# KumarRobotics/top_down_renderer

Measured on AMD Instinct MI355X. Metric: particle-updates/sec (render+score+resample), higher is better.
Workload: dtype f32

## Files before the change

### include/tdr.h

```cpp
#ifndef TDR_H_
#define TDR_H_

#include <stddef.h>
#include <stdint.h>

#ifdef __cplusplus
extern "C" {
#endif

#define TDR_OK 0
#define TDR_ERR_ARG (-1)
#define TDR_ERR_HIP (-2)
#define TDR_ERR_NOMEM (-3)

#define TDR_MAX_CLASSES 15
#define TDR_ST_FIELDS 7
enum { TDR_ST_INIT_X = 0, TDR_ST_INIT_Y = 1, TDR_ST_DX = 2, TDR_ST_DY = 3, TDR_ST_THETA = 4, TDR_ST_SCALE = 5,
       TDR_ST_HAVE_INIT = 6 };

typedef struct tdr_state {
  float init_x_px, init_y_px, dx_m, dy_m, theta, scale;
  uint8_t have_init;
  uint8_t pad_[3];
} tdr_state;
// ... 152 lines not shown

#define TDR_UW_INFO_FLOATS 65536
int tdr_k_update_weights(const float* raw_w, const float* last_dist, int64_t n, float* w_out, float* info_out,
                         void* stream);

int tdr_config_prefix_small(int on);
int64_t tdr_prefix_workspace_bytes(int64_t n);
int tdr_k_prefix(const float* w, int64_t n, float* runmax_out, void* workspace, void* stream);
int tdr_k_prefix_mode(const float* w, int64_t n, int mode, float* runmax_out, float* prefix_out, void* workspace,
                      void* stream);
int tdr_k_resample(const float* runmax, int64_t n, int64_t n_new, float shift, int64_t i_begin, int64_t i_end,
                   int32_t* idx_out, void* stream);
int tdr_k_resample_dev(const float* runmax, int64_t n, int64_t n_new, const float* shift_dev, int64_t i_begin, int64_t i_end,
                       int32_t* idx_out, void* stream);
int tdr_k_gather_states(const float* src, int64_t src_cap, int64_t src_shard, const int32_t* idx, int64_t n_new,
                        float* dst, int64_t dst_cap, void* stream);

int tdr_k_shard_pack2(const float* a, const float* b, int64_t nl, float* out, void* stream);
int tdr_k_shard_unpack2(const float* in, int world, int64_t nl, float* a_glob, float* b_glob, void* stream);
int tdr_k_unshard_states(const float* in, int world, int64_t nl, float* st, int64_t cap, void* stream);

int tdr_k_local_map_polar(const tdr_map_desc* map, const float* tab, int nb, int nr, float cx, float cy, float scale,
                          float res, float* dists_out, uint8_t* mask_out, void* stream);
int tdr_k_local_map_cart(const tdr_map_desc* map, int rows, int cols, float cx, float cy, float rot, float res,
                         float* dists_out, uint8_t* mask_out, void* stream);

int tdr_k_active_diffs(const tdr_map_desc* map, const float* tab, int nb, int nr, float res, const float* centres,
                       const int32_t* shifts, int K, int ncand, double* sums_out, void* stream);
int tdr_active_candidates_host(const float* preds, int K, int nb, float* centres, float* dists, float* thetas,
                               int32_t* shifts, int* ntheta_out, int* ndist_out);

#define TDR_MEAN_COV_FLOATS 4800
int tdr_k_mean_cov(const float* st, int64_t cap, int64_t n, const float* about, float* out, void* stream);
int tdr_k_set_scale(float* st, int64_t cap, int64_t n, const float* scale_dev, void* stream);
int tdr_k_save_ml_state(const float* info, const float* st, int64_t cap, int64_t src_shard, int64_t n, float* out12,
                        void* stream);
int tdr_k_shift_init(float* st, int64_t cap, int64_t n, float dx, float dy, void* stream);
int tdr_k_resample_gather(const float* runmax, int64_t n, int64_t n_new, const float* shift_dev, float shift,
                          int64_t i_begin, int64_t i_end, int32_t* idx_out, const float* src, int64_t src_cap,
                          int64_t src_shard, float* dst, int64_t dst_cap, const float* info, float* out12, void* stream);

int tdr_config_compact(int on);
int tdr_config_shift_uniform(int mode);
float tdr_config_shift_uniform_span(float cells);
int tdr_config_ray_split(int k);
int tdr_config_cart_skip(int on);
int tdr_config_init_mfma(int on);
int tdr_config_uw_waves(int on);
int64_t tdr_shift_uniform_launches(void);

int tdr_profile_enable(int on);
int tdr_profile_score_ms(double* total_ms, int64_t* launches);
int tdr_profile_shares(double* dense_ms, double* scattered_ms, int64_t* scattered_particles);
int tdr_profile_variants(int64_t out[16]);
int tdr_profile_ray_gate(int64_t out[4]);
int tdr_profile_su_list(int64_t out[2]);

int64_t tdr_config_tuning(const char* name, int64_t value);
int tdr_su_tail_plan(int nchunks, int k, int q, int row, int* group, int* s0, int* s1);
size_t tdr_k_su_order_workspace_ints(int64_t n, int nb);
int64_t tdr_k_su_order_slots(int64_t n, int nb);
int tdr_k_su_order(const float* st, int64_t cap, int64_t n, const int32_t* perm, int nb, float span, int32_t* workspace,
                   int32_t* slots_out, int32_t* keys_out, int32_t* counts_out, int* bucket_out, void* stream);
int tdr_k_score_prep(const tdr_map_desc* map, const float* tab, const float* scan_pk, int nb, int nr, float res,
                     const float* st, int64_t cap, int64_t n, int64_t n_total, const int32_t* perm, float uniform_scale,
                     float span, float* workspace, tdr_score_ctx* ctx, int64_t* layout, void* const* out, void* stream);
int tdr_k_score_prep_full_mask(const tdr_map_desc* map, int nb, int nr, int64_t n, int64_t n_total, const float* workspace,
                               uint32_t* out, int64_t* words, void* stream);
int tdr_selftest_score(void);
int tdr_k_selftest_round(const float* x, int64_t n, float limit, int32_t* out, void* stream);
int tdr_libm_variant(void);
int tdr_libm_force_variant(int variant);
int tdr_sincosf_host(const float* x, int64_t n, int variant, float* sin_out, float* cos_out);
int tdr_k_selftest_sincos(const float* x, int64_t n, float* sin_out, float* cos_out, void* stream);
int tdr_logf_host(const float* x, int64_t n, float* out);
int tdr_k_selftest_logf(const float* x, int64_t n, float* out, void* stream);
int tdr_k_selftest_atan2(const float* y, const float* x, int64_t n, float* out, void* stream);

int tdr_k_states_aos_to_soa(const tdr_state* aos, int64_t n, float* st, int64_t cap, void* stream);
int tdr_k_states_soa_to_aos(const float* st, int64_t cap, int64_t n, tdr_state* aos, void* stream);
size_t tdr_locality_tmp_ints(int64_t n, int map_rows, int map_cols);
int tdr_k_locality_order(const float* st, int64_t cap, int64_t n, int map_rows, int map_cols, int32_t* perm_out,
                         int32_t* keys_tmp, void* stream);
size_t tdr_locality_pose_tmp_ints(int64_t n);
int tdr_k_locality_order_pose(const float* st, int64_t cap, int64_t n, int map_rows, int map_cols, float theta_radius,
                              int32_t* perm_out, int32_t* keys_tmp, void* stream);

typedef struct tdr_map tdr_map;
typedef struct tdr_renderer tdr_renderer;
typedef struct tdr_filter tdr_filter;

int tdr_map_create(tdr_map** out);
void tdr_map_destroy(tdr_map* m);
int tdr_map_set(tdr_map* m, const float* class_maps, const uint8_t* class_mask, int ncls, int rows, int cols,
                float resolution, int center_x, int center_y);
int tdr_map_set_labels(tdr_map* m, const uint8_t* label_img, int img_h, int img_w, const int32_t* flatten_lut,
                       int lut_size, int ncls, float resolution, int center_x, int center_y);
int tdr_map_update_labels_incremental(tdr_map* m, const uint8_t* label_img, int img_h, int img_w,
                                      const int32_t* flatten_lut, int lut_size, int ncls, float resolution, int center_x,
                                      int center_y, int64_t* changed_cells);
int tdr_map_patch_labels(tdr_map* m, const uint8_t* patch, int y0, int x0, int h, int w, int center_x, int center_y,
                         int64_t* changed_cells);
int tdr_map_get_desc(const tdr_map* m, tdr_map_desc* out);
int tdr_map_sample_pts_polar(tdr_map* m, int nb, int nr, float ang_res);
int tdr_map_polar_shape(const tdr_map* m, int* nb, int* nr);
int tdr_map_set_window(tdr_map* m, int rows, int cols);
int tdr_map_window_shape(const tdr_map* m, int* rows, int* cols);
int tdr_map_info(const tdr_map* m, int* ncls, int* rows, int* cols, float* resolution, int* have_map);
int tdr_map_center(const tdr_map* m, int* center_x, int* center_y);
int tdr_map_local_map(tdr_map* m, int polar, float cx, float cy, float scale_or_rot, float res, int rows, int cols,
                      float* dists_out, uint8_t* mask_out);
int tdr_map_classes_at_point(const tdr_map* m, int px, int py, uint32_t* class_bits);
int tdr_map_best_rel_pos(tdr_map* m, const float* preds, int K, float best_rel_pos[2], float* best_diff);
int tdr_map_local_geo_map(tdr_map* m, int polar, float cx, float cy, float scale_or_rot, float res, int rows, int cols,
                          float* dists_out);
int tdr_map_load_cache(tdr_map* m, const char* cache_dir, const char* map_path, int num_classes, float resolution,
                       int center_x, int center_y, int* loaded);
int tdr_map_save_cache(tdr_map* m, const char* cache_dir, const char* map_path);
int tdr_map_save_rasters(tdr_map* m, const char* dir);
int tdr_png_read_gray8_host(const char* path, uint8_t* px_out, int64_t capacity, int* w, int* h);
int tdr_png_write_gray8_host(const char* path, const uint8_t* px, int w, int h);
int tdr_map_load_rasters(tdr_map* m, const char* dir, int num_classes, float resolution, int center_x, int center_y);
#define TDR_SVG_NO_KEY 0xFFFFFFFFu
int tdr_svg_parse_host(const char* path, float size_out[2], int64_t* n_poly, int64_t* n_vert, uint32_t* keys_out,
                       int64_t* offsets_out, float* verts_out);
int tdr_map_load_polygons(tdr_map* m, const float* verts, const int64_t* poly_offsets, const int32_t* poly_class,
                          int64_t n_poly, int width, int height, int num_classes, const int32_t* exclusive, int n_excl,
                          float resolution, int center_x, int center_y, uint8_t* planes_out);
int tdr_polygon_planes(const float* verts, const int64_t* poly_offsets, const int32_t* poly_class, int64_t n_poly,
                       int width, int height, int num_classes, const int32_t* exclusive, int n_excl, float resolution,
                       uint8_t* planes_out);
int tdr_map_load_svg(tdr_map* m, const char* path, const uint32_t* fill_keys, const int32_t* flatten_lut, int lut_size,
                     int num_classes, const int32_t* exclusive, int n_excl, float resolution, int center_x, int center_y);
int tdr_png_read_color_host(const char* path, uint8_t* bgr_out, int64_t capacity, int* w, int* h);
int tdr_map_load_color_image(tdr_map* m, const uint8_t* bgr, int img_h, int img_w, const uint32_t* fill_keys,
                             const int32_t* flatten_lut, int lut_size, int num_classes, float resolution, int center_x,
                             int center_y);
int tdr_map_load_color_png(tdr_map* m, const char* path, const uint32_t* fill_keys, const int32_t* flatten_lut,
                           int lut_size, int num_classes, float resolution, int center_x, int center_y);

int tdr_renderer_create(const int32_t* flatten_lut256, tdr_renderer** out);
void tdr_renderer_destroy(tdr_renderer* r);
int tdr_renderer_render(tdr_renderer* r, int polar, const float* pts, int stride, int ioff, int64_t n, float res,
                        float ang_res, int ncls, int rows, int cols, float* imgs_out);

int tdr_renderer_render_geo(tdr_renderer* r, int polar, const float* pts, int stride, int64_t width, int64_t height,
                            float res, float ang_res, int rows, int cols, float* imgs_out);

#define TDR_COMM_ID_BYTES 128
typedef struct tdr_comm tdr_comm;
typedef struct tdr_comm_ops {
  void* ctx;
  int (*all_gather)(void* ctx, const void* send_dev, void* recv_dev, size_t bytes_per_rank, void* stream);
  int (*broadcast)(void* ctx, void* buf_dev, size_t bytes, int root, void* stream);
} tdr_comm_ops;
int tdr_comm_rccl_unique_id(void* id_out128);
int tdr_comm_create_rccl(int world_size, int rank, const void* unique_id128, tdr_comm** out);
int tdr_comm_create(int world_size, int rank, const tdr_comm_ops* ops, tdr_comm** out);
void tdr_comm_destroy(tdr_comm* c);
int tdr_comm_world(const tdr_comm* c);
int tdr_comm_rank(const tdr_comm* c);
int tdr_comm_all_gather(tdr_comm* c, const void* send_dev, void* recv_dev, size_t bytes_per_rank, void* stream);
int tdr_comm_broadcast(tdr_comm* c, void* buf_dev, size_t bytes, int root, void* stream);
int tdr_filter_create_sharded(tdr_map* map, int n_max, const tdr_filter_params* fp, uint32_t seed, tdr_comm* comm,
                              tdr_filter** out);
int64_t tdr_filter_num_local(const tdr_filter* f);
// ... 280 lines not shown
```

### top_down_renderer_amd/_lib.py

```python
import ctypes as C
import os

_PKG = os.path.dirname(os.path.abspath(__file__))
SO_PATH = os.environ.get("TDR_LIB_PATH") or os.path.join(_PKG, "libtdr_hip.so")

TDR_ST_FIELDS = 7
TDR_MAX_CLASSES = 15
TDR_SVG_NO_KEY = 0xFFFFFFFF


class FilterParamsC(C.Structure):
    _fields_ = [
        ("pos_cov", C.c_float), ("theta_cov", C.c_float), ("regularization", C.c_float),
        ("init_pos_px_x", C.c_float), ("init_pos_px_y", C.c_float), ("init_pos_px_cov", C.c_float),
        ("init_pos_m_x", C.c_float), ("init_pos_m_y", C.c_float),
        ("init_pos_deg_theta", C.c_float), ("init_pos_deg_cov", C.c_float),
        ("force_on_map", C.c_int32),
        ("fixed_scale", C.c_float), ("scale_log_min", C.c_float), ("scale_log_max", C.c_float),
        ("num_classes", C.c_int32),
        ("class_weights", C.c_float * 16),
    ]


class MapDescC(C.Structure):
# ... 308 lines not shown
    "tdr_filter_get_resample_indices": (_i, [_vp, _vp, _i64]),
    "tdr_filter_mean_cov": (_i, [_vp, _i, _vp, _vp]),
    "tdr_filter_freeze_scale": (_i, [_vp]),
    "tdr_filter_is_scale_frozen": (_i, [_vp]),
    "tdr_filter_scale": (_f, [_vp]),
    "tdr_filter_num_particles": (_i64, [_vp]),
    "tdr_filter_update_map": (_i, [_vp, _vp, _vp, _i, _i, _i, _f, _i, _i]),
    "tdr_batch_step": (_i, [_vp, _i, _vp, _vp]),
    "tdr_batch_last_stats": (_i, [_vp, _vp]),
    "tdr_batch_render_polar": (_i, [_vp, _i, _vp, _f, _i, _i, _i, _vp]),
    "tdr_renderer_get_render": (_i, [_vp, _vp, _vp]),
    "tdr_batch_pose": (_i, [_vp, _i, _vp, _vp]),
    "tdr_viz_plane_words": (C.c_size_t, [_i, _i]),
    "tdr_viz_arrow_host": (_i, [_i, _i, _vp]),
    "tdr_viz_overlay_host": (_i, [_vp, _vp, _i, _vp, _vp, _i, _i, _vp, _i, C.POINTER(_i)]),
    "tdr_k_viz_particles": (_i, [_vp, _i64, _i64, _i, _i, _vp, _vp]),
    "tdr_k_viz_segments": (_i, [_vp, _i, _i, _i, _vp, _vp]),
    "tdr_k_viz_compose": (_i, [_vp, _i, _i, _vp, _i, _i, _vp, _vp]),
    "tdr_filter_set_viz_background": (_i, [_vp, _vp, _i, _i]),
    "tdr_filter_visualize": (_i, [_vp, _f, _vp, _i, _vp, _i64, C.POINTER(_i), C.POINTER(_i)]),
    "tdr_k_viz_particles_jobs": (_i, [_vp, _i, _i64, _vp]),
    "tdr_k_viz_segments_jobs": (_i, [_vp, _i, _i, _vp]),
    "tdr_k_viz_compose_jobs": (_i, [_vp, _i, _i64, _vp]),
    "tdr_batch_visualize": (_i, [_vp, _i, _f, _vp, _vp]),
    "tdr_k_viz_compose_fleet": (_i, [_vp, _i, _vp, _vp, _i, _i, _vp, _i, _i, _vp, _vp]),
    "tdr_map_set_viz_background": (_i, [_vp, _vp, _i, _i]),
    "tdr_map_set_viz_background_labels": (_i, [_vp, _vp, _i, _i, _vp]),
    "tdr_batch_visualize_fleet": (_i, [_vp, _i, _f, _vp, _vp, _i, _vp, _i64, C.POINTER(_i), C.POINTER(_i), _vp]),
    "tdr_k_scan_picture": (_i, [_vp, _i, _i64, _vp, _vp, _vp, _vp]),
    "tdr_k_analog_picture": (_i, [_vp, _i64, _f, _vp, _vp]),
    "tdr_k_label_picture": (_i, [_vp, _i64, _vp, _vp, _vp]),
    "tdr_k_scan_picture_jobs": (_i, [_vp, _i, _i64, _vp, _i, _vp, _vp]),
    "tdr_k_analog_picture_jobs": (_i, [_vp, _i, _i64, _f, _vp]),
    "tdr_k_label_picture_jobs": (_i, [_vp, _i, _i64, _vp, _vp]),
    "tdr_renderer_visualize": (_i, [_vp, _vp, _vp, _vp, _i64, C.POINTER(_i), C.POINTER(_i)]),
    "tdr_renderer_visualize_analog": (_i, [_vp, _i, _f, _vp, _i64, C.POINTER(_i), C.POINTER(_i)]),
    "tdr_scan_picture_host": (_i, [_vp, _i, _i, _i, _vp, _vp, _vp]),
    "tdr_filter_set_viz_background_labels": (_i, [_vp, _vp, _i, _i, _vp]),
    "tdr_batch_scan_pictures": (_i, [_vp, _i, _vp, _vp, _vp, _vp]),
    "tdr_k_fuse_votes_jobs": (_i, [_vp, _vp, _i, _i, _vp, _i, _i64, _vp, _vp, _vp, _vp]),
    "tdr_k_fuse_votes": (_i, [_vp, _vp, _i, _i, _vp, _i, _i, _i, _f, _f, _f, _f, _f, _vp, _vp, _vp, _vp]),
    "tdr_k_fuse_labels": (_i, [_vp, _i, _i, _i, _i, _i, _f, _vp, _u32, _u32, _u32, _vp, _vp, _vp, _i, _vp, _vp]),
    "tdr_k_fuse_decay": (_i, [_vp, _i, _i, _i, _i, _vp, _vp]),
    "tdr_fuser_create": (_i, [_vp, _vp, _u32, _u32, _u32, C.POINTER(_vp)]),
    "tdr_fuser_destroy": (None, [_vp]),
    "tdr_fuser_add": (_i, [_vp, _vp, _f, _f, _f, _f, _f, C.POINTER(_u64), C.POINTER(_u64)]),
    "tdr_fuser_add_batch": (_i, [_vp, _vp, _i, _vp, C.POINTER(_u64), C.POINTER(_u64)]),
    "tdr_fuser_add_images": (_i, [_vp, _vp, _i, _i, _i, _f, _f, _f, _f, _f, C.POINTER(_u64), C.POINTER(_u64)]),
    "tdr_fuser_apply": (_i, [_vp, _vp, _i, C.POINTER(_i64)]),
    "tdr_fuser_decay": (_i, [_vp, _i]),
    "tdr_fuser_reset": (_i, [_vp]),
    "tdr_fuser_rebase": (_i, [_vp, C.POINTER(_i)]),
    "tdr_fuser_get_votes": (_i, [_vp, _vp]),
    "tdr_fuser_get_labels": (_i, [_vp, _vp]),
    "tdr_fuser_stats": (_i, [_vp, _vp]),
    "tdr_kld_workspace_bytes": (C.c_size_t, [_i64]),
    "tdr_k_kld_keys": (_i, [_vp, _i64, _i64, C.POINTER(KldParamsC), _vp, _vp]),
    "tdr_k_kld_count": (_i, [_vp, _i64, _i64, C.POINTER(KldParamsC), _vp, _vp, _vp]),
    "tdr_k_kld_count_jobs": (_i, [_vp, _i, C.POINTER(KldParamsC), _vp]),
    "tdr_kld_bound_host": (_i64, [_i64, C.c_double, C.c_double]),
    "tdr_kld_target_host": (_i64, [_i64, _i64, _i64, _i64]),
    "tdr_filter_kld_count": (_i, [_vp, C.POINTER(KldParamsC), C.POINTER(_i64), C.POINTER(_i64), C.POINTER(_i64)]),
    "tdr_batch_kld_count": (_i, [_vp, _i, C.POINTER(KldParamsC), _vp, _vp, _vp, _vp]),
    "tdr_philox4x32_host": (None, [_vp, _vp, _vp]),
    "tdr_inject_threshold_host": (_u32, [C.c_double]),
    "tdr_recovery_track_host": (C.c_double, [C.POINTER(RecoveryStateC), C.c_double, C.POINTER(RecoveryParamsC)]),
    "tdr_recovery_reset_host": (None, [C.POINTER(RecoveryStateC)]),
    "tdr_map_road_workspace_bytes": (C.c_size_t, [_i, _i]),
    "tdr_k_map_road_cells": (_i, [_vp, _vp, _vp, _vp, _vp]),
    "tdr_k_inject": (_i, [_vp, _i64, _i64, _i64, _vp, _vp, _i64, _u64, _u64, _u32, _i, _vp, _vp]),
    "tdr_k_inject_jobs": (_i, [_vp, _i, _vp]),
    "tdr_map_road_cells": (_i, [_vp, C.POINTER(_vp), C.POINTER(_i64)]),
    "tdr_map_read_road_cells": (_i, [_vp, _vp, _i64, C.POINTER(_i64)]),
    "tdr_filter_get_weight_stats": (_i, [_vp, _vp]),
    "tdr_filter_inject": (_i, [_vp, C.c_double, _i, _u64, C.POINTER(_i64)]),
    "tdr_filter_recovery_step": (_i, [_vp, C.POINTER(RecoveryStateC), C.POINTER(RecoveryParamsC), C.POINTER(C.c_double),
                                      C.POINTER(_i64)]),
    "tdr_batch_inject": (_i, [_vp, _i, _vp, _i, _vp, _vp, _vp]),
    "tdr_set_error": (_i, [_i, C.c_char_p]),
    "tdr_locality_tmp_ints": (C.c_size_t, [_i64, _i, _i]),
    "tdr_locality_pose_tmp_ints": (C.c_size_t, [_i64]),
    "tdr_k_locality_order_pose": (_i, [_vp, _i64, _i64, _i, _i, _f, _vp, _vp, _vp]),
    "tdr_k_locality_order": (_i, [_vp, _i64, _i64, _i, _i, _vp, _vp, _vp]),
}

_lib = None


class TdrError(RuntimeError):
    pass


def load():
    global _lib
    if _lib is not None:
        return _lib
    if not os.path.exists(SO_PATH):
        raise TdrError(
            f"{SO_PATH} is missing: build the HIP extension first (python -m top_down_renderer_amd.build, or "
            "__graft_entry__.build()).  There is no CPU fallback.")
    L = C.CDLL(SO_PATH)
    for name, (res, args) in SIGNATURES.items():
        fn = getattr(L, name)
        fn.restype = res
        fn.argtypes = args
    _lib = L
    return L


def check(rc):
    if rc != 0:
        raise TdrError(f"libtdr_hip error {rc}: {load().tdr_last_error().decode()}")
```

### top_down_renderer_amd/csrc/tdr_config.cpp

```cpp
#include "tdr_config.h"

#include <algorithm>
#include <cstring>

#include "tdr_score_su.h"

namespace {
TdrConfig g_cfg;
thread_local const TdrConfig* t_override = nullptr;

int as_int(int64_t v) { return (int)std::max<int64_t>(v, -1); }
int64_t set_flag(int& m, int64_t v) {
  if (as_int(v) >= 0) m = as_int(v) ? 1 : 0;
  return m;
}
int64_t set_from_0(int& m, int64_t v, int hi) {
  if (v >= 0) m = (int)std::min<int64_t>(v, hi);
  return m;
}

struct Knob {
  const char* name;
  int64_t (*set)(TdrConfig& c, int64_t v);
};
const Knob kKnobs[] = {
    {"score_waves", [](TdrConfig& c, int64_t v) { if (v > 0) c.score_waves = v; return c.score_waves; }},
    {"score_group", [](TdrConfig& c, int64_t v) -> int64_t { if (v >= 0) c.score_group = (int)v; return c.score_group; }},
    {"su_group", [](TdrConfig& c, int64_t v) -> int64_t { if (v >= 0) c.su_group = (int)v; return c.su_group; }},
    {"batch_init_search", [](TdrConfig& c, int64_t v) { return set_flag(c.batch_init_search, v); }},
    {"init_ahead", [](TdrConfig& c, int64_t v) -> int64_t { if (v >= 1) c.init_ahead = (int)std::min<int64_t>(v, 3); return c.init_ahead; }},
    {"prefix_head", [](TdrConfig& c, int64_t v) -> int64_t { if (as_int(v) >= 0) c.pfx_head = std::min(std::max(as_int(v), 1), PFX_HEAD); return c.pfx_head; }},
    {"ray_borrow", [](TdrConfig& c, int64_t v) { return set_flag(c.ray_borrow, v); }},
    {"ray_patch", [](TdrConfig& c, int64_t v) { return set_flag(c.ray_patch, v); }},
    {"ray_block_major", [](TdrConfig& c, int64_t v) { return set_flag(c.ray_block_major, v); }},
    {"cart_seg_rows", [](TdrConfig& c, int64_t v) -> int64_t { if (as_int(v) >= 0) c.cart_seg_rows = as_int(v) - as_int(v) % 4; return c.cart_seg_rows; }},
    {"mt_stretches", [](TdrConfig& c, int64_t v) { return set_flag(c.mt_stretches, v); }},
    {"su_tail_groups", [](TdrConfig& c, int64_t v) { return set_from_0(c.su_tail_groups, v, 1 << 20); }},
    {"su_tail_parts", [](TdrConfig& c, int64_t v) -> int64_t {
       if (v >= 0) c.su_tail_parts = v >= 8 ? 8 : (v >= 4 ? 4 : (v >= 2 ? 2 : 1));
       return c.su_tail_parts;
     }},
    {"su_order_bucket", [](TdrConfig& c, int64_t v) { return set_flag(c.su_order_bucket, v); }},
    {"su_full_list", [](TdrConfig& c, int64_t v) { return set_flag(c.su_full_list, v); }},
    {"init_device",[](TdrConfig& c, int64_t v) { return set_flag(c.init_device, v); }},
    {"init_window_words", [](TdrConfig& c, int64_t v) {
       if (v > 0) c.init_window = std::min<int64_t>((v + INI_TILE - 1) / INI_TILE * INI_TILE, (int64_t)INI_TILE * INI_MAX_TILES);
       return c.init_window;
     }},
    {"cart_init_chunk", [](TdrConfig& c, int64_t v) { if (v >= 1) c.cart_init_chunk = std::min<int64_t>(v, 1 << 24); return c.cart_init_chunk; }},
};
}

const TdrConfig& tdr_cfg() { return t_override ? *t_override : g_cfg; }
TdrConfigScope::TdrConfigScope(const TdrConfig& c) : cfg_(c), outer_(t_override) { t_override = &cfg_; }
TdrConfigScope::~TdrConfigScope() { t_override = outer_; }

extern "C" {
int64_t tdr_config_tuning(const char* name, int64_t value) {
  if (!name) return -1;
  for (const Knob& k : kKnobs)
    if (std::strcmp(name, k.name) == 0) return k.set(g_cfg, value);
  return -1;
}
int tdr_config_compact(int on) { return (int)set_flag(g_cfg.use_compact, on); }
int tdr_config_shift_uniform(int mode) { return (int)set_from_0(g_cfg.su_mode, mode, 2); }
float tdr_config_shift_uniform_span(float cells) {
  if (cells >= 0.f) { g_cfg.su_span = cells; g_cfg.su_span_fixed = true; }
  else if (cells < -1.5f) { g_cfg.su_span = TdrConfig{}.su_span; g_cfg.su_span_fixed = false; }
  return g_cfg.su_span;
}
int tdr_config_ray_split(int k) { return (int)set_from_0(g_cfg.ray_split, k, TDR_RAY_MAX_SPLIT); }
int tdr_config_cart_skip(int on) { return (int)set_flag(g_cfg.cart_skip, on); }
int tdr_config_init_mfma(int on) { return (int)set_flag(g_cfg.init_mfma, on); }
int tdr_config_uw_waves(int on) { return (int)set_flag(g_cfg.uw_waves, on); }
int tdr_config_prefix_small(int on) { return (int)set_flag(g_cfg.pfx_small, on); }
int64_t tdr_config_rec16_min_particles(int64_t n) {
  if (n >= 0) g_cfg.rec16_min = n;
  return g_cfg.rec16_min;
}
}
```

### top_down_renderer_amd/csrc/tdr_config.h

```cpp
#ifndef TDR_CONFIG_H_
#define TDR_CONFIG_H_
#include <cstdint>

struct TdrConfig {
  int su_mode = 1;
  float su_span = 16.f;
  bool su_span_fixed = false;
  int su_group = 0;
  int su_tail_groups = 4, su_tail_parts = 4;
  int su_order_bucket = 1;
  int su_full_list = 1;
  int ray_split = 0;
  int ray_borrow = 1;
  int ray_patch = 1;
  int ray_block_major = 1;
  int cart_skip = 1;
  int cart_seg_rows = 32;
  int64_t cart_init_chunk = 4096;
  int use_compact = 1;
  int64_t score_waves = 131072;
  int score_group = 0;
  int init_mfma = 1;
  int init_ahead = 1;
  int64_t rec16_min = 8192;
  int batch_init_search = 0;
  int init_device = 1;
  int64_t init_window = 1 << 21;
  int pfx_small = 1;
  int pfx_head = 64;
  int uw_waves = 1;
  int mt_stretches = 1;
};

const TdrConfig& tdr_cfg();

class TdrConfigScope {
 public:
  explicit TdrConfigScope(const TdrConfig& c);
  ~TdrConfigScope();
  TdrConfigScope(const TdrConfigScope&) = delete;
  TdrConfigScope& operator=(const TdrConfigScope&) = delete;

 private:
  TdrConfig cfg_;
  const TdrConfig* outer_;
};
#endif
```

### top_down_renderer_amd/csrc/tdr_filter.hip

```cpp
#include <random>

#include <rocprim/device/device_radix_sort.hpp>
using TdrSortConfig = rocprim::radix_sort_config<rocprim::default_config, rocprim::merge_sort_config<512, 512, 4>, rocprim::default_config>;

#include "tdr_common.h"
#include "tdr_filter_dev.h"

__device__ __forceinline__ uint32_t mulhi32(uint32_t a, uint32_t b) { return __umulhi(a, b); }
__device__ void philox4x32_10(uint32_t c[4], uint32_t k0, uint32_t k1) {
#pragma unroll
  for (int r = 0; r < 10; r++) {
    uint32_t hi0 = mulhi32(0xD2511F53u, c[0]), lo0 = 0xD2511F53u * c[0];
    uint32_t hi1 = mulhi32(0xCD9E8D57u, c[2]), lo1 = 0xCD9E8D57u * c[2];
    uint32_t n0 = hi1 ^ c[1] ^ k0, n1 = lo1, n2 = hi0 ^ c[3] ^ k1, n3 = lo0;
    c[0] = n0; c[1] = n1; c[2] = n2; c[3] = n3;
    k0 += 0x9E3779B9u; k1 += 0xBB67AE85u;
  }
}

__global__ void propagate_kernel(float* __restrict__ st, int64_t cap, int64_t n, float* __restrict__ last_dist,
                                 float tx, float ty, float omega, int scale_freeze, float pos_cov, float theta_cov,
                                 const float* __restrict__ z4, uint64_t seed, uint64_t step, int64_t index_base,
                                 int libm_fma) {
  const int64_t p = (int64_t)blockIdx.x * blockDim.x + threadIdx.x;
// ... 526 lines not shown
__global__ void unshard_states_kernel(const float* __restrict__ in, int world, int64_t nl, float* __restrict__ st,
                                      int64_t cap) {
  const int64_t g = (int64_t)blockIdx.x * blockDim.x + threadIdx.x;
  if (g >= (int64_t)world * nl) return;
  const int64_t r = g / nl, l = g - r * nl;
#pragma unroll
  for (int f = 0; f < TDR_ST_FIELDS; f++) st[f * cap + g] = in[(r * TDR_ST_FIELDS + f) * nl + l];
}
extern "C" int tdr_k_shard_pack2(const float* a, const float* b, int64_t nl, float* out, void* stream) {
  if (!a || !b || !out || nl < 0) return fail(TDR_ERR_ARG, "shard_pack2: bad arguments");
  if (nl == 0) return TDR_OK;
  hipLaunchKernelGGL(shard_pack2_kernel, dim3((unsigned)cdiv(nl, 256)), dim3(256), 0, (hipStream_t)stream, a, b, nl, out);
  LAUNCH_CHECK("shard_pack2");
  return TDR_OK;
}
extern "C" int tdr_k_shard_unpack2(const float* in, int world, int64_t nl, float* a_glob, float* b_glob, void* stream) {
  if (!in || !a_glob || !b_glob || world < 1 || nl < 0) return fail(TDR_ERR_ARG, "shard_unpack2: bad arguments");
  if (nl == 0) return TDR_OK;
  hipLaunchKernelGGL(shard_unpack2_kernel, dim3((unsigned)cdiv((int64_t)world * nl, 256)), dim3(256), 0,
                     (hipStream_t)stream, in, world, nl, a_glob, b_glob);
  LAUNCH_CHECK("shard_unpack2");
  return TDR_OK;
}
extern "C" int tdr_k_unshard_states(const float* in, int world, int64_t nl, float* st, int64_t cap, void* stream) {
  if (!in || !st || world < 1 || nl < 0 || cap < (int64_t)world * nl) return fail(TDR_ERR_ARG, "unshard_states: bad arguments");
  if (nl == 0) return TDR_OK;
  hipLaunchKernelGGL(unshard_states_kernel, dim3((unsigned)cdiv((int64_t)world * nl, 256)), dim3(256), 0,
                     (hipStream_t)stream, in, world, nl, st, cap);
  LAUNCH_CHECK("unshard_states");
  return TDR_OK;
}

__global__ void aos_to_soa_kernel(const tdr_state* __restrict__ aos, int64_t n, float* __restrict__ st, int64_t cap) {
  const int64_t p = (int64_t)blockIdx.x * blockDim.x + threadIdx.x;
  if (p >= n) return;
  const tdr_state s = aos[p];
  st[TDR_ST_INIT_X * cap + p] = s.init_x_px;
  st[TDR_ST_INIT_Y * cap + p] = s.init_y_px;
  st[TDR_ST_DX * cap + p] = s.dx_m;
  st[TDR_ST_DY * cap + p] = s.dy_m;
  st[TDR_ST_THETA * cap + p] = s.theta;
  st[TDR_ST_SCALE * cap + p] = s.scale;
  st[TDR_ST_HAVE_INIT * cap + p] = s.have_init ? 1.f : 0.f;
}
__global__ void soa_to_aos_kernel(const float* __restrict__ st, int64_t cap, int64_t n, tdr_state* __restrict__ aos) {
  const int64_t p = (int64_t)blockIdx.x * blockDim.x + threadIdx.x;
  if (p >= n) return;
  tdr_state s;
  s.init_x_px = st[TDR_ST_INIT_X * cap + p];
  s.init_y_px = st[TDR_ST_INIT_Y * cap + p];
  s.dx_m = st[TDR_ST_DX * cap + p];
  s.dy_m = st[TDR_ST_DY * cap + p];
  s.theta = st[TDR_ST_THETA * cap + p];
  s.scale = st[TDR_ST_SCALE * cap + p];
  s.have_init = st[TDR_ST_HAVE_INIT * cap + p] != 0.f;
  s.pad_[0] = s.pad_[1] = s.pad_[2] = 0;
  aos[p] = s;
}
extern "C" int tdr_k_states_aos_to_soa(const tdr_state* aos, int64_t n, float* st, int64_t cap, void* stream) {
  if (!aos || !st || n < 0 || cap < n) return fail(TDR_ERR_ARG, "aos_to_soa: bad arguments");
  if (n == 0) return TDR_OK;
  hipLaunchKernelGGL(aos_to_soa_kernel, dim3((unsigned)cdiv(n, 256)), dim3(256), 0, (hipStream_t)stream, aos, n, st,
                     cap);
  LAUNCH_CHECK("aos_to_soa");
  return TDR_OK;
}
extern "C" int tdr_k_states_soa_to_aos(const float* st, int64_t cap, int64_t n, tdr_state* aos, void* stream) {
  if (!aos || !st || n < 0 || cap < n) return fail(TDR_ERR_ARG, "soa_to_aos: bad arguments");
  if (n == 0) return TDR_OK;
  hipLaunchKernelGGL(soa_to_aos_kernel, dim3((unsigned)cdiv(n, 256)), dim3(256), 0, (hipStream_t)stream, st, cap, n,
                     aos);
  LAUNCH_CHECK("soa_to_aos");
  return TDR_OK;
}

__device__ __forceinline__ uint32_t spread_bits16(uint32_t v) {
  v &= 0xFFFFu;
  v = (v | (v << 8)) & 0x00FF00FFu;
  v = (v | (v << 4)) & 0x0F0F0F0Fu;
  v = (v | (v << 2)) & 0x33333333u;
  v = (v | (v << 1)) & 0x55555555u;
  return v;
}
__global__ void loc_key_kernel(const float* __restrict__ st, int64_t cap, int64_t n, float xmax, float ymax,
                               uint32_t* __restrict__ keys, int32_t* __restrict__ vals) {
  const int64_t p = (int64_t)blockIdx.x * blockDim.x + threadIdx.x;
  if (p >= n) return;
  const float sc = st[TDR_ST_SCALE * cap + p];
  float cx = st[TDR_ST_DX * cap + p] * sc + st[TDR_ST_INIT_X * cap + p];
  float cy = st[TDR_ST_DY * cap + p] * sc + st[TDR_ST_INIT_Y * cap + p];
  if (!(cx == cx)) cx = 0.f;
  if (!(cy == cy)) cy = 0.f;
  const uint32_t hx = (uint32_t)fminf(fmaxf(cx * 2.f, 0.f), xmax);
  const uint32_t hy = (uint32_t)fminf(fmaxf(cy * 2.f, 0.f), ymax);
  keys[p] = spread_bits16(hx) | (spread_bits16(hy) << 1);
  vals[p] = (int32_t)p;
}

__device__ __forceinline__ uint64_t spread_bits21_3(uint64_t v) {
  v &= 0x1FFFFFull;
  v = (v | (v << 32)) & 0x1F00000000FFFFull;
  v = (v | (v << 16)) & 0x1F0000FF0000FFull;
  v = (v | (v << 8)) & 0x100F00F00F00F00Full;
  v = (v | (v << 4)) & 0x10C30C30C30C30C3ull;
  v = (v | (v << 2)) & 0x1249249249249249ull;
  return v;
}
__global__ void loc_key_pose_kernel(const float* __restrict__ st, int64_t cap, int64_t n, float xmax, float ymax,
                                    float theta_step, uint64_t* __restrict__ keys, int32_t* __restrict__ vals) {
  const int64_t p = (int64_t)blockIdx.x * blockDim.x + threadIdx.x;
  if (p >= n) return;
  const float sc = st[TDR_ST_SCALE * cap + p];
  float cx = st[TDR_ST_DX * cap + p] * sc + st[TDR_ST_INIT_X * cap + p];
  float cy = st[TDR_ST_DY * cap + p] * sc + st[TDR_ST_INIT_Y * cap + p];
  float th = st[TDR_ST_THETA * cap + p];
  if (!(cx == cx)) cx = 0.f;
  if (!(cy == cy)) cy = 0.f;
  if (!(fabsf(th) < 1e6f)) th = 0.f;
  th = th - 6.2831855f * floorf(th / 6.2831855f);
  const uint64_t hx = (uint64_t)fminf(fmaxf(cx * 2.f, 0.f), xmax);
  const uint64_t hy = (uint64_t)fminf(fmaxf(cy * 2.f, 0.f), ymax);
  const uint64_t ht = (uint64_t)fminf(fmaxf(th / theta_step, 0.f), 2097151.f);
  keys[p] = spread_bits21_3(hx) | (spread_bits21_3(hy) << 1) | (spread_bits21_3(ht) << 2);
  vals[p] = (int32_t)p;
}
static size_t radix_tmp_bytes64(int64_t n) {
  size_t bytes = 0;
  uint64_t* k = nullptr;
  int32_t* v = nullptr;
  hipError_t e = rocprim::radix_sort_pairs(nullptr, bytes, k, k, v, v, (size_t)n, 0u, 63u, (hipStream_t)0, false);
  if (e != hipSuccess || bytes == 0) bytes = (size_t)(n + 4096) * 32;
  return bytes;
}
extern "C" size_t tdr_locality_pose_tmp_ints(int64_t n) {
  if (n < 1) n = 1;
  return (size_t)(5 * n + 64) + (radix_tmp_bytes64(n) + 3) / 4 + 64;
}
extern "C" int tdr_k_locality_order_pose(const float* st, int64_t cap, int64_t n, int map_rows, int map_cols,
                                         float theta_radius, int32_t* perm_out, int32_t* keys_tmp, void* stream) {
  if (!st || !perm_out || !keys_tmp || n < 0 || cap < n || map_rows < 1 || map_cols < 1 || !(theta_radius > 0.f))
    return fail(TDR_ERR_ARG, "locality_order_pose: bad arguments");
  if (map_rows > 1000000 || map_cols > 1000000) return fail(TDR_ERR_ARG, "locality_order_pose: map too large");
  if (n == 0) return TDR_OK;
  hipStream_t s = (hipStream_t)stream;
  uint64_t* keys_in = reinterpret_cast<uint64_t*>(keys_tmp);
  uint64_t* keys_out = keys_in + n;
  int32_t* vals_in = keys_tmp + 4 * n;
  void* tmp = keys_tmp + 5 * n + 64 - ((5 * n) % 64);
  size_t tmp_bytes = radix_tmp_bytes64(n);
  hipLaunchKernelGGL(loc_key_pose_kernel, dim3((unsigned)cdiv(n, 256)), dim3(256), 0, s, st, cap, n,
                     (float)(2 * map_cols - 1), (float)(2 * map_rows - 1), 0.5f / theta_radius, keys_in, vals_in);
  LAUNCH_CHECK("loc_key_pose");
  HIP_TRY(rocprim::radix_sort_pairs(tmp, tmp_bytes, keys_in, keys_out, vals_in, perm_out, (size_t)n, 0u, 63u, s, false));
  return TDR_OK;
}

static size_t radix_tmp_bytes(int64_t n) {
  size_t bytes = 0;
  uint32_t* k = nullptr;
  int32_t* v = nullptr;
  hipError_t e = rocprim::radix_sort_pairs<TdrSortConfig>(nullptr, bytes, k, k, v, v, (size_t)n, 0u, 32u, (hipStream_t)0, false);
  if (e != hipSuccess || bytes == 0) bytes = (size_t)(n + 4096) * 16;
  return bytes;
}

extern "C" size_t tdr_locality_tmp_ints(int64_t n, int map_rows, int map_cols) {
  (void)map_rows; (void)map_cols;
  if (n < 1) n = 1;
  return (size_t)(3 * n + 64) + (radix_tmp_bytes(n) + 3) / 4 + 64;
}

extern "C" int tdr_k_locality_order(const float* st, int64_t cap, int64_t n, int map_rows, int map_cols,
                                    int32_t* perm_out, int32_t* keys_tmp, void* stream) {
  if (!st || !perm_out || !keys_tmp || n < 0 || cap < n || map_rows < 1 || map_cols < 1)
    return fail(TDR_ERR_ARG, "locality_order: bad arguments");
  if (map_rows > 32767 || map_cols > 32767) return fail(TDR_ERR_ARG, "locality_order: map larger than 32767 px");
  if (n == 0) return TDR_OK;
  hipStream_t s = (hipStream_t)stream;
  uint32_t* keys_in = reinterpret_cast<uint32_t*>(keys_tmp);
  uint32_t* keys_out = keys_in + n;
  int32_t* vals_in = keys_tmp + 2 * n;
  void* tmp = keys_tmp + 3 * n + 64 - ((3 * n) % 64);
  size_t tmp_bytes = radix_tmp_bytes(n);
  hipLaunchKernelGGL(loc_key_kernel, dim3((unsigned)cdiv(n, 256)), dim3(256), 0, s, st, cap, n,
                     (float)(2 * map_cols - 1), (float)(2 * map_rows - 1), keys_in, vals_in);
  LAUNCH_CHECK("loc_key");
  unsigned bits = 2;
  while ((1u << (bits / 2)) < (unsigned)(2 * std::max(map_rows, map_cols)) && bits < 32) bits += 2;
  HIP_TRY(rocprim::radix_sort_pairs<TdrSortConfig>(tmp, tmp_bytes, keys_in, keys_out, vals_in, perm_out, (size_t)n, 0u, bits, s,
                                    false));
  return TDR_OK;
}
```

Baseline: 25.91 million.

## Replace rocprim radix sort with custom fused key+histogram LSD radix sort for locality order

Adds a custom LSD radix sort for the Morton-key locality ordering, used for mid-sized particle counts. The first histogram is fused into the key-generation kernel, and each pass uses at most 64 blocks with 9-bit digits, wave-level ballot matching for ranks, and a per-block prefix over a small count table. The aim is to cut rocprim's launch count and temporary-buffer overhead for small sorts. It also narrows the pose-sort bit range from 63 bits to 3x the needed coordinate width. The cost is more hand-written code and a larger workspace reservation.

```diff
diff --git a/include/tdr.h b/include/tdr.h
--- a/include/tdr.h
+++ b/include/tdr.h
@@ -258,6 +258,7 @@
 size_t tdr_locality_tmp_ints(int64_t n, int map_rows, int map_cols);
 int tdr_k_locality_order(const float* st, int64_t cap, int64_t n, int map_rows, int map_cols, int32_t* perm_out,
                          int32_t* keys_tmp, void* stream);
+int tdr_locality_order_plan(int64_t n, int map_rows, int map_cols, int* block_out, int* digits_out);
 size_t tdr_locality_pose_tmp_ints(int64_t n);
 int tdr_k_locality_order_pose(const float* st, int64_t cap, int64_t n, int map_rows, int map_cols, float theta_radius,
                               int32_t* perm_out, int32_t* keys_tmp, void* stream);
diff --git a/top_down_renderer_amd/_lib.py b/top_down_renderer_amd/_lib.py
--- a/top_down_renderer_amd/_lib.py
+++ b/top_down_renderer_amd/_lib.py
@@ -414,6 +414,7 @@
     "tdr_locality_pose_tmp_ints": (C.c_size_t, [_i64]),
     "tdr_k_locality_order_pose": (_i, [_vp, _i64, _i64, _i, _i, _f, _vp, _vp, _vp]),
     "tdr_k_locality_order": (_i, [_vp, _i64, _i64, _i, _i, _vp, _vp, _vp]),
+    "tdr_locality_order_plan": (_i, [_i64, _i, _i, C.POINTER(_i), C.POINTER(_i)]),
 }
 
 _lib = None
diff --git a/top_down_renderer_amd/csrc/tdr_config.cpp b/top_down_renderer_amd/csrc/tdr_config.cpp
--- a/top_down_renderer_amd/csrc/tdr_config.cpp
+++ b/top_down_renderer_amd/csrc/tdr_config.cpp
@@ -41,6 +41,7 @@
        return c.su_tail_parts;
      }},
     {"su_order_bucket", [](TdrConfig& c, int64_t v) { return set_flag(c.su_order_bucket, v); }},
+    {"loc_order_radix", [](TdrConfig& c, int64_t v) { return set_flag(c.loc_order_radix, v); }},
     {"su_full_list", [](TdrConfig& c, int64_t v) { return set_flag(c.su_full_list, v); }},
     {"init_device",[](TdrConfig& c, int64_t v) { return set_flag(c.init_device, v); }},
     {"init_window_words", [](TdrConfig& c, int64_t v) {
diff --git a/top_down_renderer_amd/csrc/tdr_config.h b/top_down_renderer_amd/csrc/tdr_config.h
--- a/top_down_renderer_amd/csrc/tdr_config.h
+++ b/top_down_renderer_amd/csrc/tdr_config.h
@@ -9,6 +9,7 @@
   int su_group = 0;
   int su_tail_groups = 4, su_tail_parts = 4;
   int su_order_bucket = 1;
+  int loc_order_radix = 1;
   int su_full_list = 1;
   int ray_split = 0;
   int ray_borrow = 1;
diff --git a/top_down_renderer_amd/csrc/tdr_filter.hip b/top_down_renderer_amd/csrc/tdr_filter.hip
--- a/top_down_renderer_amd/csrc/tdr_filter.hip
+++ b/top_down_renderer_amd/csrc/tdr_filter.hip
@@ -632,10 +632,7 @@
   v = (v | (v << 1)) & 0x55555555u;
   return v;
 }
-__global__ void loc_key_kernel(const float* __restrict__ st, int64_t cap, int64_t n, float xmax, float ymax,
-                               uint32_t* __restrict__ keys, int32_t* __restrict__ vals) {
-  const int64_t p = (int64_t)blockIdx.x * blockDim.x + threadIdx.x;
-  if (p >= n) return;
+__device__ __forceinline__ uint32_t loc_key(const float* __restrict__ st, int64_t cap, int64_t p, float xmax, float ymax) {
   const float sc = st[TDR_ST_SCALE * cap + p];
   float cx = st[TDR_ST_DX * cap + p] * sc + st[TDR_ST_INIT_X * cap + p];
   float cy = st[TDR_ST_DY * cap + p] * sc + st[TDR_ST_INIT_Y * cap + p];
@@ -643,8 +640,135 @@
   if (!(cy == cy)) cy = 0.f;
   const uint32_t hx = (uint32_t)fminf(fmaxf(cx * 2.f, 0.f), xmax);
   const uint32_t hy = (uint32_t)fminf(fmaxf(cy * 2.f, 0.f), ymax);
-  keys[p] = spread_bits16(hx) | (spread_bits16(hy) << 1);
+  return spread_bits16(hx) | (spread_bits16(hy) << 1);
+}
+__global__ void loc_key_kernel(const float* __restrict__ st, int64_t cap, int64_t n, float xmax, float ymax,
+                               uint32_t* __restrict__ keys, int32_t* __restrict__ vals) {
+  const int64_t p = (int64_t)blockIdx.x * blockDim.x + threadIdx.x;
+  if (p >= n) return;
+  keys[p] = loc_key(st, cap, p, xmax, ymax);
   vals[p] = (int32_t)p;
+}
+
+constexpr int LOC_COLS = 512;
+constexpr int LOC_WAVES = LOC_COLS / 64;
+constexpr int LOC_MAX_BLOCKS = 64;
+constexpr int LOC_MAX_DIGITS = 4;
+constexpr int64_t LOC_RADIX_MIN = 2048, LOC_RADIX_MAX = (int64_t)LOC_MAX_BLOCKS * 8192;
+
+__global__ __launch_bounds__(LOC_COLS) void loc_key_hist_kernel(const float* __restrict__ st, int64_t cap, int64_t n,
+                                                                float xmax, float ymax, int B, uint32_t mask0,
+                                                                uint32_t* __restrict__ keys, int32_t* __restrict__ vals,
+                                                                int* __restrict__ tab) {
+  __shared__ int hist[LOC_COLS];
+  hist[threadIdx.x] = 0;
+  __syncthreads();
+  const int64_t p0 = (int64_t)blockIdx.x * B;
+#pragma unroll 2
+  for (int o = threadIdx.x; o < B; o += LOC_COLS) {
+    const int64_t p = p0 + o;
+    if (p < n) {
+      const uint32_t key = loc_key(st, cap, p, xmax, ymax);
+      keys[p] = key;
+      vals[p] = (int32_t)p;
+      atomicAdd(&hist[key & mask0], 1);
+    }
+  }
+  __syncthreads();
+  tab[blockIdx.x * LOC_COLS + threadIdx.x] = hist[threadIdx.x];
+}
+__global__ __launch_bounds__(LOC_COLS) void loc_count_kernel(const uint32_t* __restrict__ keys, int64_t n, int B, int shift,
+                                                             uint32_t mask, int* __restrict__ tab) {
+  __shared__ int hist[LOC_COLS];
+  hist[threadIdx.x] = 0;
+  __syncthreads();
+  const int64_t p0 = (int64_t)blockIdx.x * B;
+#pragma unroll 4
+  for (int o = threadIdx.x; o < B; o += LOC_COLS)
+    if (p0 + o < n) atomicAdd(&hist[(keys[p0 + o] >> shift) & mask], 1);
+  __syncthreads();
+  tab[blockIdx.x * LOC_COLS + threadIdx.x] = hist[threadIdx.x];
+}
+
+__device__ __forceinline__ uint64_t loc_match(uint32_t v, int bits, bool live) {
+  uint64_t same = __ballot(live);
+  for (int b = 0; b < bits; b++) {
+    const bool one = (v >> b) & 1u;
+    const uint64_t ones = __ballot(one);
+    same &= one ? ones : ~ones;
+  }
+  return same;
+}
+
+template <int IPT, bool LAST>
+__global__ __launch_bounds__(LOC_COLS) void loc_pass_kernel(const uint32_t* __restrict__ keys_in, const int32_t* __restrict__ vals_in,
+                                                            int64_t n, const int* __restrict__ tab, int blocks, int shift,
+                                                            int dbits, uint32_t* __restrict__ keys_out,
+                                                            int32_t* __restrict__ vals_out) {
+  constexpr int B = IPT * LOC_COLS;
+  __shared__ int ctr[LOC_WAVES][LOC_COLS];
+  __shared__ int wave_sum[LOC_WAVES];
+  const int d = threadIdx.x, lane = d & 63, w = d >> 6, b = blockIdx.x;
+  const int64_t t0 = (int64_t)b * B + (int64_t)w * (IPT * 64) + lane;
+  uint32_t key[IPT];
+  int32_t val[IPT];
+  int rank[IPT];
+#pragma unroll
+  for (int it = 0; it < IPT; it++) {
+    const int64_t t = t0 + it * 64;
+    key[it] = t < n ? keys_in[t] : 0u;
+    val[it] = t < n ? vals_in[t] : 0;
+  }
+#pragma unroll
+  for (int u = 0; u < LOC_WAVES; u++) ctr[u][d] = 0;
+  int total = 0, before = 0;
+#pragma unroll 8
+  for (int r = 0; r < blocks; r++) {
+    const int c = tab[r * LOC_COLS + d];
+    total += c;
+    before += r < b ? c : 0;
+  }
+  int incl = total;
+#pragma unroll
+  for (int o = 1; o < 64; o <<= 1) {
+    const int v = __shfl_up(incl, o);
+    if (lane >= o) incl += v;
+  }
+  if (lane == 63) wave_sum[w] = incl;
+  __syncthreads();
+  int base = incl - total + before;
+  for (int u = 0; u < w; u++) base += wave_sum[u];
+  const uint32_t dmask = (1u << dbits) - 1u;
+#pragma unroll
+  for (int it = 0; it < IPT; it++) {
+    const bool live = t0 + it * 64 < n;
+    const uint32_t dg = (key[it] >> shift) & dmask;
+    const uint64_t same = loc_match(dg, dbits, live);
+    const int below = __popcll(same & (((uint64_t)1 << lane) - 1)), all = __popcll(same);
+    const int at = live ? ctr[w][dg] : 0;
+    if (live && below == all - 1) ctr[w][dg] = at + all;
+    __builtin_amdgcn_fence(__ATOMIC_RELEASE, "wavefront");
+    __builtin_amdgcn_wave_barrier();
+    rank[it] = at + below;
+  }
+  __syncthreads();
+  int run = base;
+#pragma unroll
+  for (int u = 0; u < LOC_WAVES; u++) {
+    const int c = ctr[u][d];
+    ctr[u][d] = run;
+    run += c;
+  }
+  __syncthreads();
+#pragma unroll
+  for (int it = 0; it < IPT; it++) {
+    const uint32_t dg = (key[it] >> shift) & dmask;
+    const uint32_t q = (uint32_t)(ctr[w][dg] + rank[it]);
+    if (t0 + it * 64 < n && (int64_t)q < n) {
+      if (!LAST) keys_out[q] = key[it];
+      vals_out[q] = val[it];
+    }
+  }
 }
 
 __device__ __forceinline__ uint64_t spread_bits21_3(uint64_t v) {
@@ -698,10 +822,14 @@
   int32_t* vals_in = keys_tmp + 4 * n;
   void* tmp = keys_tmp + 5 * n + 64 - ((5 * n) % 64);
   size_t tmp_bytes = radix_tmp_bytes64(n);
-  hipLaunchKernelGGL(loc_key_pose_kernel, dim3((unsigned)cdiv(n, 256)), dim3(256), 0, s, st, cap, n,
-                     (float)(2 * map_cols - 1), (float)(2 * map_rows - 1), 0.5f / theta_radius, keys_in, vals_in);
+  const float xmax = (float)(2 * map_cols - 1), ymax = (float)(2 * map_rows - 1), theta_step = 0.5f / theta_radius;
+  hipLaunchKernelGGL(loc_key_pose_kernel, dim3((unsigned)cdiv(n, 256)), dim3(256), 0, s, st, cap, n, xmax, ymax, theta_step,
+                     keys_in, vals_in);
   LAUNCH_CHECK("loc_key_pose");
-  HIP_TRY(rocprim::radix_sort_pairs(tmp, tmp_bytes, keys_in, keys_out, vals_in, perm_out, (size_t)n, 0u, 63u, s, false));
+  const uint64_t top = std::max({(uint64_t)xmax, (uint64_t)ymax, (uint64_t)fminf(6.2831855f / theta_step + 1.f, 2097151.f)});
+  unsigned width = 1;
+  while (width < 21 && (top >> width) != 0) width++;
+  HIP_TRY(rocprim::radix_sort_pairs(tmp, tmp_bytes, keys_in, keys_out, vals_in, perm_out, (size_t)n, 0u, 3u * width, s, false));
   return TDR_OK;
 }
 
@@ -714,10 +842,71 @@
   return bytes;
 }
 
+static unsigned loc_key_bits(int map_rows, int map_cols) {
+  unsigned bits = 2;
+  while ((1u << (bits / 2)) < (unsigned)(2 * std::max(map_rows, map_cols)) && bits < 32) bits += 2;
+  return bits;
+}
+
+struct LocPlan {
+  int B, blocks, digits;
+  int width[LOC_MAX_DIGITS], shift[LOC_MAX_DIGITS];
+};
+static bool loc_radix_plan(int64_t n, int map_rows, int map_cols, LocPlan* p) {
+  if (!tdr_cfg().loc_order_radix || n <= LOC_RADIX_MIN || n > LOC_RADIX_MAX) return false;
+  p->B = 1024;
+  while (cdiv(n, p->B) > LOC_MAX_BLOCKS) p->B *= 2;
+  p->blocks = (int)cdiv(n, p->B);
+  const int bits = (int)loc_key_bits(map_rows, map_cols);
+  p->digits = (bits + 8) / 9;
+  for (int j = 0, at = 0; j < p->digits; j++) {
+    p->width[j] = bits / p->digits + (j < bits % p->digits ? 1 : 0);
+    p->shift[j] = at;
+    at += p->width[j];
+  }
+  return true;
+}
+extern "C" int tdr_locality_order_plan(int64_t n, int map_rows, int map_cols, int* block_out, int* digits_out) {
+  LocPlan p;
+  if (map_rows < 1 || map_cols < 1 || map_rows > 32767 || map_cols > 32767 || !loc_radix_plan(n, map_rows, map_cols, &p)) return 0;
+  if (block_out) *block_out = p.B;
+  if (digits_out) *digits_out = p.digits;
+  return 1;
+}
+static int64_t loc_pad64(int64_t n) { return (n + 63) / 64 * 64; }
+static size_t loc_radix_reserve(int64_t n) {
+  if (n <= LOC_RADIX_MIN) return 0;
+  return (size_t)(4 * loc_pad64(std::min(n, LOC_RADIX_MAX)) + (int64_t)LOC_MAX_BLOCKS * LOC_COLS);
+}
+
 extern "C" size_t tdr_locality_tmp_ints(int64_t n, int map_rows, int map_cols) {
   (void)map_rows; (void)map_cols;
   if (n < 1) n = 1;
-  return (size_t)(3 * n + 64) + (radix_tmp_bytes(n) + 3) / 4 + 64;
+  return std::max((size_t)(3 * n + 64) + (radix_tmp_bytes(n) + 3) / 4 + 64, loc_radix_reserve(n));
+}
+
+template <int IPT>
+static int loc_radix_passes(const LocPlan& P, int64_t n, uint32_t* keys_a, uint32_t* keys_b, int32_t* vals_a, int32_t* vals_b,
+                            int* tab, int32_t* perm_out, hipStream_t s) {
+  for (int j = 0; j < P.digits; j++) {
+    if (j > 0) {
+      hipLaunchKernelGGL(loc_count_kernel, dim3((unsigned)P.blocks), dim3(LOC_COLS), 0, s, (const uint32_t*)keys_a, n, P.B,
+                         P.shift[j], (1u << P.width[j]) - 1u, tab);
+      LAUNCH_CHECK("loc_count");
+    }
+    if (j == P.digits - 1) {
+      hipLaunchKernelGGL((loc_pass_kernel<IPT, true>), dim3((unsigned)P.blocks), dim3(LOC_COLS), 0, s, (const uint32_t*)keys_a,
+                         (const int32_t*)vals_a, n, (const int*)tab, P.blocks, P.shift[j], P.width[j], (uint32_t*)nullptr,
+                         perm_out);
+    } else {
+      hipLaunchKernelGGL((loc_pass_kernel<IPT, false>), dim3((unsigned)P.blocks), dim3(LOC_COLS), 0, s, (const uint32_t*)keys_a,
+                         (const int32_t*)vals_a, n, (const int*)tab, P.blocks, P.shift[j], P.width[j], keys_b, vals_b);
+      std::swap(keys_a, keys_b);
+      std::swap(vals_a, vals_b);
+    }
+    LAUNCH_CHECK("loc_pass");
+  }
+  return TDR_OK;
 }
 
 extern "C" int tdr_k_locality_order(const float* st, int64_t cap, int64_t n, int map_rows, int map_cols,
@@ -727,17 +916,33 @@
   if (map_rows > 32767 || map_cols > 32767) return fail(TDR_ERR_ARG, "locality_order: map larger than 32767 px");
   if (n == 0) return TDR_OK;
   hipStream_t s = (hipStream_t)stream;
+  const float xmax = (float)(2 * map_cols - 1), ymax = (float)(2 * map_rows - 1);
+  LocPlan P;
+  if (loc_radix_plan(n, map_rows, map_cols, &P)) {
+    const int64_t np = loc_pad64(n);
+    uint32_t* keys_a = reinterpret_cast<uint32_t*>(keys_tmp);
+    uint32_t* keys_b = keys_a + np;
+    int32_t* vals_a = keys_tmp + 2 * np;
+    int32_t* vals_b = keys_tmp + 3 * np;
+    int* tab = keys_tmp + 4 * np;
+    hipLaunchKernelGGL(loc_key_hist_kernel, dim3((unsigned)P.blocks), dim3(LOC_COLS), 0, s, st, cap, n, xmax, ymax, P.B,
+                       (1u << P.width[0]) - 1u, keys_a, vals_a, tab);
+    LAUNCH_CHECK("loc_key_hist");
+    switch (P.B) {
+      case 1024: return loc_radix_passes<2>(P, n, keys_a, keys_b, vals_a, vals_b, tab, perm_out, s);
+      case 2048: return loc_radix_passes<4>(P, n, keys_a, keys_b, vals_a, vals_b, tab, perm_out, s);
+      case 4096: return loc_radix_passes<8>(P, n, keys_a, keys_b, vals_a, vals_b, tab, perm_out, s);
+      default: return loc_radix_passes<16>(P, n, keys_a, keys_b, vals_a, vals_b, tab, perm_out, s);
+    }
+  }
   uint32_t* keys_in = reinterpret_cast<uint32_t*>(keys_tmp);
   uint32_t* keys_out = keys_in + n;
   int32_t* vals_in = keys_tmp + 2 * n;
   void* tmp = keys_tmp + 3 * n + 64 - ((3 * n) % 64);
   size_t tmp_bytes = radix_tmp_bytes(n);
-  hipLaunchKernelGGL(loc_key_kernel, dim3((unsigned)cdiv(n, 256)), dim3(256), 0, s, st, cap, n,
-                     (float)(2 * map_cols - 1), (float)(2 * map_rows - 1), keys_in, vals_in);
+  hipLaunchKernelGGL(loc_key_kernel, dim3((unsigned)cdiv(n, 256)), dim3(256), 0, s, st, cap, n, xmax, ymax, keys_in, vals_in);
   LAUNCH_CHECK("loc_key");
-  unsigned bits = 2;
-  while ((1u << (bits / 2)) < (unsigned)(2 * std::max(map_rows, map_cols)) && bits < 32) bits += 2;
-  HIP_TRY(rocprim::radix_sort_pairs<TdrSortConfig>(tmp, tmp_bytes, keys_in, keys_out, vals_in, perm_out, (size_t)n, 0u, bits, s,
-                                    false));
-  return TDR_OK;
-}
+  HIP_TRY(rocprim::radix_sort_pairs<TdrSortConfig>(tmp, tmp_bytes, keys_in, keys_out, vals_in, perm_out, (size_t)n, 0u,
+                                                   loc_key_bits(map_rows, map_cols), s, false));
+  return TDR_OK;
+}
```

Result: no change. 26.06 million, median of 6 (+0.5%).
